# francois141/nori-ray-tracer

Measured on AMD Instinct MI355X. Metric: Msamples/sec on cbox_path_mis 512×512@512spp; per-pixel L2 vs CPU ref, higher is better.
Workload: dtype f32; 1 GPU; cbox_path_mis 512x512@512spp; scene=scenes/pa4/cbox/cbox_path_mis.xml, integrator=path_mis, parallelism=single GPU

## Files before the change

include/nori_gpu.h:

```cpp
#ifndef NORI_GPU_H
#define NORI_GPU_H

#ifndef __HIPCC_RTC__
#include <stddef.h>
#endif
#include <stdint.h>

#ifdef __cplusplus
extern "C" {
#endif

#define NORI_GPU_ABI_VERSION 7

#define NORI_OK               0
#define NORI_ERR_INVALID     -1
#define NORI_ERR_IO          -2
#define NORI_ERR_PARSE       -3
#define NORI_ERR_UNSUPPORTED -4
#define NORI_ERR_HIP         -5
#define NORI_ERR_CANCELLED   -6
#define NORI_ERR_OOM         -7

enum { NORI_SHAPE_MESH = 0 , NORI_SHAPE_SPHERE = 1  };
enum {
// ... 172 lines not shown
int nori_read_exr(const char *path, int *width, int *height, float *rgb);
int nori_read_image(const char *path, int *width, int *height, uint8_t *rgb);

typedef struct nori_bvh_info {
    uint32_t ref_nodes;
    uint32_t device_nodes;
    uint32_t depth;
    uint32_t num_prims;
    float sah_cost;
    uint32_t pad;
    uint64_t order_hash;
} nori_bvh_info;
int nori_scene_bvh_info(const nori_scene_desc *scene, nori_bvh_info *out);

typedef struct nori_scan_info {
    uint32_t records;
    uint32_t pairs;
    uint32_t plane_end[3];
    uint32_t tris;
} nori_scan_info;
int nori_scene_scan_list(const nori_scene_desc *scene, nori_scan_info *info, float *records, float *plane_c,
                         float *plane_f);

int nori_scene_scan_rtc(const nori_scene_desc *scene, const char *arch, size_t *code_bytes, double *ms);

int nori_scene_shade_rtc(const nori_scene_desc *scene, const char *arch, size_t *code_bytes, double *ms);

typedef struct nori_gpu_ctx nori_gpu_ctx;

typedef struct nori_gpu_render_desc {
    uint32_t pass_begin;
    uint32_t pass_count;
    uint32_t num_blocks;
    const uint32_t *block_ids;
    uint64_t seed;
    int32_t output_on_device;
    uint32_t path_pool;
    int32_t timing;
    float *variance_out;
} nori_gpu_render_desc;

typedef struct nori_gpu_stats {
    uint64_t samples;
    uint64_t invalid_samples;
    uint64_t rays_closest;
    uint64_t rays_shadow;
// ... 170 lines not shown
```

nori-ray-tracer_amd/csrc/kernels.h:

```cpp
#pragma once
#include <hip/hip_runtime.h>

#include <string>
#include <vector>

#include "film_put.h"
#include "kernel_config.h"

namespace nori {

constexpr int kTraceBlock = 128;
constexpr int kTraceSpill = 64;
#ifndef NORI_STACK_KEYS
#define NORI_STACK_KEYS 1
#endif
constexpr int stack_lds_entries(int stack) { return NORI_STACK_KEYS ? stack / 2 : stack; }
constexpr int kSplatBlock = 256;
#ifndef NORI_SCATTER_ROWS
#define NORI_SCATTER_ROWS 1
#endif
#ifndef NORI_SCAN_RAYS
#define NORI_SCAN_RAYS 2
#endif
constexpr int kScanRays = NORI_SCAN_RAYS;
#ifndef NORI_SCAN_RAYS_SHADOW
#define NORI_SCAN_RAYS_SHADOW 1
#endif
constexpr int kScanRaysShadow = NORI_SCAN_RAYS_SHADOW;

struct SplatDesc {
    uint32_t M;
    uint32_t passes;
    uint32_t pass_begin;
    uint32_t passes_per_wg;
    const int4 *blocks;
    uint64_t seed;
    float *var;
};

struct ScanRtcScene {
    const float *rec;
    uint32_t nrec;
    const float *plane_c, *plane_f;
    uint32_t pairs;
    uint32_t plane_end[3];
    uint32_t tris, real;
};
struct ScanRtc {
    hipModule_t mod = nullptr;
    hipFunction_t extend = nullptr, shadow = nullptr, trace[2] = {nullptr, nullptr};
    hipFunction_t both = nullptr;
    int k_extend = 0;
    double compile_ms = 0.0;
    bool cached = false;
    size_t code_bytes = 0;
};
struct ShadeRtc {
    hipModule_t mod = nullptr;
    hipFunction_t shade = nullptr;
    int integrator = 0;
    bool lds = false;
    double compile_ms = 0.0;
    bool cached = false;
    size_t code_bytes = 0;
};
constexpr bool kShadeRtcDefault = true;
std::string rtc_const_scene(const ScanRtcScene &sc);
bool rtc_compile(const ScanRtcScene &sc, const std::string &arch, int trace_cull, std::vector<char> &code, double &ms,
                 bool &cached, std::string &why, bool fresh = false);
// ... 91 lines not shown
```

nori-ray-tracer_amd/csrc/rtc.hip:

```cpp
#include <dlfcn.h>
#include <sys/stat.h>
#include <unistd.h>

#include <cerrno>
#include <chrono>
#include <cstdio>
#include <cstdlib>
#include <cstring>
#include <map>
#include <mutex>
#include <string>
#include <vector>

#include "kernels.h"
#include "rtc_cache.h"
#include "shade_kernel.h"

namespace nori {

#include "rtc_headers.inc"

namespace {

bool rtc_debug() {
// ... 219 lines not shown

bool rtc_off() {
    const char *e = std::getenv("NORI_RTC");
    return e && e[0] == '0';
}

}

int rtc_rays_per_thread() {
    const char *e = std::getenv("NORI_RTC_K");
    const int k = e ? std::atoi(e) : 1;
    return k == 1 || k == 2 || k == 4 ? k : 1;
}

std::string rtc_const_scene(const ScanRtcScene &sc) {
    std::string s = "#pragma once\n";
    s += "constexpr uint32_t kCPlaneEnd[3] = {" + std::to_string(sc.plane_end[0]) + "u, " +
         std::to_string(sc.plane_end[1]) + "u, " + std::to_string(sc.plane_end[2]) + "u};\n";
    s += "constexpr uint32_t kCTris = " + std::to_string(sc.tris) + "u, kCReal = " + std::to_string(sc.real) +
         "u, kCPrims = " + std::to_string(sc.nrec) + "u;\n";
    s += "constexpr float kCRec[] = {" + flt_list(sc.rec, 12 * (size_t)sc.nrec) + "};\n";
    s += "constexpr float kCPlaneF[] = {" + flt_list(sc.plane_f, 8 * (size_t)sc.pairs) + "};\n";
    s += "constexpr float kCPlaneC[] = {" + flt_list(sc.plane_c, sc.pairs) + "};\n";
    return s;
}

bool rtc_compile(const ScanRtcScene &sc, const std::string &arch, int trace_cull, std::vector<char> &code,
                 double &ms, bool &cached, std::string &why, bool fresh) {
    const int k = rtc_rays_per_thread();
    const char *wv = std::getenv("NORI_RTC_WAVES");
    RtcJob job{"scan_", "nori_scan_rtc.hip", kProgram, rtc_const_scene(sc), {
        "--offload-arch=" + arch, "-O3", "-std=c++17", "-ffp-contract=off", "-fno-slp-vectorize",
        "-munsafe-fp-atomics", "-DNORI_CONST_SCENE=1", "-DNORI_RTC_K=" + std::to_string(k),
        "-DNORI_RTC_WAVES=" + std::to_string(wv ? std::atoi(wv) : 0),
        "-DNORI_RTC_KS=" + std::to_string(kScanRaysShadow), "-DNORI_EXTEND_BLOCK=" + std::to_string(NORI_EXTEND_BLOCK),
        "-DNORI_SHADOW_BLOCK=" + std::to_string(NORI_SHADOW_BLOCK), "-DNORI_RTC_TRACE_BLOCK=" + std::to_string(kTraceBlock),
        "-DNORI_SCAN_GROUP=" + std::to_string(kScanGroup), "-DNORI_TRACE_GROUP=" + std::to_string(kTraceGroup),
        "-DNORI_SPHERE_FAST=" + std::to_string(NORI_SPHERE_FAST), "-DNORI_RTC_TRACE_CULL=" + std::to_string(trace_cull)}};
    return rtc_run(job, fresh, code, ms, cached, why);
}

bool rtc_compile_shade(const ScanRtcScene &sc, const std::string &arch, int integrator, bool lds,
                       std::vector<char> &code, double &ms, bool &cached, std::string &why, bool fresh) {
    RtcJob job{"shade_", "nori_shade_rtc.hip", kShadeProgram, rtc_const_scene(sc), {
        "--offload-arch=" + arch, "-O3", "-std=c++17", "-ffp-contract=off", "-fno-slp-vectorize",
        "-munsafe-fp-atomics", "-DNORI_CONST_SCENE=1", "-DNORI_RTC_INTEG=" + std::to_string(integrator),
// ... 130 lines not shown
```

nori-ray-tracer_amd/csrc/scan.h:

```cpp
#pragma once
#include "dev_scene.h"

namespace nori {

#define INF_F __builtin_inff()

struct TRay {
    V3 o, d, rcp;
    float mint, maxt;
};

ND bool box_test(const float4 &mn, const float4 &mx, const TRay &r, float &tnear) {
    bool ok = true;
    float nearT = -INF_F, farT = INF_F;
#define NORI_AXIS(c)                                                            \
    {                                                                           \
        float t1 = (mn.c - r.o.c) * r.rcp.c, t2 = (mx.c - r.o.c) * r.rcp.c;      \
        float lo = t1 > t2 ? t2 : t1, hi = t1 > t2 ? t1 : t2;                   \
        bool zero = r.d.c == 0.0f;                                              \
        float n2 = smax(lo, nearT), f2 = smin(hi, farT);                        \
        ok = ok && (zero ? !(r.o.c < mn.c || r.o.c > mx.c) : (n2 <= f2));       \
        nearT = zero ? nearT : n2;                                              \
        farT = zero ? farT : f2;                                                \
    }
    NORI_AXIS(x) NORI_AXIS(y) NORI_AXIS(z)
#undef NORI_AXIS
    tnear = nearT;
    return ok && r.mint <= farT && nearT <= r.maxt;
}

ND float rcp_det(float x) { return rcp_rn(x); }
ND bool tri_hit(const float4 &a, const float4 &b, const float4 &c, const TRay &r, float &t, float &u, float &v) {
    V3 v0 = ld3(a), e1 = ld3(b), e2 = ld3(c);
    V3 pvec = cross(r.d, e2);
    float det = dot(e1, pvec);
    if (det > -1e-8f && det < 1e-8f) return false;
    float inv_det = rcp_rn(det);
    V3 tvec = r.o - v0;
    u = dot(tvec, pvec) * inv_det;
    if (u < 0.0f || u > 1.0f) return false;
    V3 qvec = cross(tvec, e1);
    v = dot(r.d, qvec) * inv_det;
    if (v < 0.0f || u + v > 1.0f) return false;
    t = dot(e2, qvec) * inv_det;
    return t >= r.mint && t <= r.maxt;
}

ND bool sphere_hit(const float4 &a, const float4 &b, const TRay &r, float &t) {
    V3 oc = r.o - ld3(a);
    float rad = b.x;
    float A = dot(r.d, r.d);
    float B = 2.0f * dot(oc, r.d);
    float C = dot(oc, oc) - rad * rad;
    float disc = (B * B - 4 * A * C);
// ... 45 lines not shown
        inv_det;
    return !(det > -1e-8f && det < 1e-8f) && !(u < 0.0f || u > 1.0f) && !(v < 0.0f || u + v > 1.0f) &&
           t >= r.mint && t <= r.maxt;
}
template <bool FAST = false>
ND bool sphere_hit_nb(const float4 &a, const float4 &b, const TRay &r, float &t) {
    V3 oc = r.o - ld3(a);
    float rad = b.x;
    float A = dot(r.d, r.d);
    float B = 2.0f * dot(oc, r.d);
    float C = dot(oc, oc) - rad * rad;
    float disc = (B * B - 4 * A * C);
    float delta = fsqrt<FAST>(B * B - 4 * A * C);
    float t1 = (-B - delta) / (2 * A), t2 = (-B + delta) / (2 * A);
    bool h1 = r.mint <= t1 && t1 <= r.maxt, h2 = r.mint <= t2 && t2 <= r.maxt;
    t = h1 ? t1 : t2;
    return (disc > 0) && (h1 || h2);
}

#ifndef NORI_SPHERE_FAST
#define NORI_SPHERE_FAST 1
#endif
ND bool in_range60(float x) { return fabsf(x) >= 0x1p-60f && fabsf(x) <= 0x1p60f; }
ND bool sphere_hit_fast(const float4 &a, const float4 &b, const TRay &r, float &t) {
    if (!NORI_SPHERE_FAST) return sphere_hit_nb(a, b, r, t);
    V3 oc = r.o - ld3(a);
    float rad = b.x;
    float A = dot(r.d, r.d);
    float B = 2.0f * dot(oc, r.d);
    float C = dot(oc, oc) - rad * rad;
    float disc = (B * B - 4 * A * C);
    const float y = 2 * A;
#ifdef __HIP_DEVICE_COMPILE__
    const float s0 = __builtin_amdgcn_sqrtf(disc);
    const float sd = __uint_as_float(__float_as_uint(s0) - 1u), su = __uint_as_float(__float_as_uint(s0) + 1u);
    const float rd = __builtin_fmaf(-sd, s0, disc), ru = __builtin_fmaf(-su, s0, disc);
    float delta = ru > 0.0f ? su : (rd <= 0.0f ? sd : s0);
    const float ry = rcp_rn(y);
    float x1 = -B - delta, x2 = -B + delta;
    float q1 = x1 * ry, q2 = x2 * ry;
    float t1 = __builtin_fmaf(__builtin_fmaf(-y, q1, x1), ry, q1), t2 = __builtin_fmaf(__builtin_fmaf(-y, q2, x2), ry, q2);
    const bool fast = disc >= 0x1p-96f && disc < 0x1p96f && in_range60(y) && in_range60(x1) && in_range60(x2);
    if (__builtin_expect(disc > 0 && !fast, 0)) {
        delta = sqrtf(B * B - 4 * A * C);
        t1 = (-B - delta) / (2 * A);
        t2 = (-B + delta) / (2 * A);
    }
#else
    float delta = sqrtf(B * B - 4 * A * C);
    float t1 = (-B - delta) / y, t2 = (-B + delta) / y;
#endif
    bool h1 = r.mint <= t1 && t1 <= r.maxt, h2 = r.mint <= t2 && t2 <= r.maxt;
    t = h1 ? t1 : t2;
    return (disc > 0) && (h1 || h2);
}

template <int K>
ND void scan_prologue(const DevScene &S, TRay (&r)[K], bool (&live)[K]) {
    const float4 rmn = make_float4(S.root_min[0], S.root_min[1], S.root_min[2], 0.f);
    const float4 rmx = make_float4(S.root_max[0], S.root_max[1], S.root_max[2], 0.f);
#pragma unroll
    for (int k = 0; k < K; ++k) {
        TRay &x = r[k];
        if (x.mint == kEps) x.mint = smax(x.mint, x.mint * smax(smax(fabsf(x.o.x), fabsf(x.o.y)), fabsf(x.o.z)));
        x.rcp = V3{rcp_full(x.d.x), rcp_full(x.d.y), rcp_full(x.d.z)};
        float tn;
        live[k] = live[k] && !(x.maxt < x.mint) && box_test(rmn, rmx, x, tn);
    }
}

constexpr float kPlaneLo = 1.0f - 0x1p-16f, kPlaneHi = 1.0f + 0x1p-16f;
ND bool plane_may_hit(float o, float d, float c, float mint, float maxt) {
    const float T = o - c, ad = fabsf(d);
    const float s = d > 0.0f ? -T : T;
    const float lo = mint > 0.0f ? mint * kPlaneLo * ad : -INF_F, hi = maxt > 0.0f ? maxt * kPlaneHi * ad : INF_F;
    return s > lo && s < hi;
}

template <int A>
ND float comp(const V3 &v) { return A == 0 ? v.x : A == 1 ? v.y : v.z; }

template <int A>
ND bool pair_candidate(const TRay &r, const float4 &f0, const float4 &f1, float mlo, float mhi, float so, float sd) {
    constexpr int B = (A + 1) % 3, C = (A + 2) % 3;
    const float tf = (f1.y - comp<A>(r.o)) * comp<A>(r.rcp);
    const float dB = __builtin_fmaf(tf, comp<B>(r.d), comp<B>(r.o) - f0.x);
    const float dC = __builtin_fmaf(tf, comp<C>(r.d), comp<C>(r.o) - f0.z);
    const float S = __builtin_fmaf(fabsf(tf), sd, so);
// ... 134 lines not shown
    }
    NORI_SC_UNROLL
    for (uint32_t i = nt; i < n; ++i) {
        if (ANY && all_done()) return;
        const float4 p0 = NORI_SC_PRIM(3 * i), p1 = NORI_SC_PRIM(3 * i + 1);
        const uint32_t pos = __float_as_uint(NORI_SC_PRIM(3 * i + 2).w);
#pragma unroll
        for (int k = 0; k < K; ++k) {
            float t = 0;
            const bool h = sphere_hit_fast(p0, p1, r[k], t);
            if (h && live[k] && (ANY || t != tb[k] || pos > lb[k])) {
                found[k] = true;
                if (!ANY) {
                    r[k].maxt = tb[k] = t;
                    ub[k] = vb[k] = 0.0f;
                    pb[k] = __float_as_uint(p0.w);
                    lb[k] = pos;
                }
            }
        }
    }
}

template <int K, bool ANY, int CULL = 1, bool ZMINT = false>
ND void scan_rays(const DevScene &S, TRay (&r)[K], bool (&live)[K], float (&tb)[K], uint32_t (&pb)[K],
                  float (&ub)[K], float (&vb)[K], bool (&found)[K]) {
    scan_core<K, ANY, CULL, ZMINT>(S, r, live, tb, pb, ub, vb, found);
}

ND void path_ray(const DevScene &S, const float4 &a, const float4 &b, TRay &r) {
    r.o = ld3(a);
    r.d = ld3(b);
    const bool cam = (__float_as_uint(b.w) & kCameraRay) != 0u;
    r.mint = cam ? S.near_clip * a.w : kEps;
    r.maxt = cam ? S.far_clip * a.w : INF_F;
}

ND void shadow_add(float4 *rec, const float4 &c) {
    const uint32_t w = __float_as_uint(c.w);
    const float4 L = rec[w];
    rec[w] = make_float4(L.x + c.x, L.y + c.y, L.z + c.z, L.w);
}

#ifndef NORI_EXTEND_BLOCK
#define NORI_EXTEND_BLOCK 256
#endif
#ifndef NORI_SHADOW_BLOCK
#define NORI_SHADOW_BLOCK 256
#endif
// ... 93 lines not shown
```

nori-ray-tracer_amd/csrc/scene_prep.cpp:

```cpp
#include "scene_prep.h"

#include <algorithm>
#include <cstdio>
#include <cstdlib>
#include <cstring>

#include "rebuild.h"

namespace nori {

std::string &last_error() {
    static thread_local std::string e;
    return e;
}
bool debug_log() {
    const char *e = std::getenv("NORI_DEBUG");
    return e && e[0] == '1';
}

static float filter_eval(const nori_camera_desc &c, float x) {
    switch (c.filter_type) {
    case NORI_FILTER_GAUSSIAN: {
        float alpha = -1.0f / (2.0f * c.filter_p0 * c.filter_p0);
        float v = std::exp(alpha * x * x) - std::exp(alpha * c.filter_radius * c.filter_radius);
// ... 247 lines not shown
            const int a = k ? C : B;
            const float mid = (float)(0.5 * (lo[a] + hi[a]));
            const double half = std::max(hi[a] - mid, mid - lo[a]);
            const double Kb = (K1 * V + 2.0 * E * gam(70) + std::ldexp(E, -23) + std::ldexp(std::fabs(mid), -22)) * 1.05;
            f[2 * k] = mid;
            f[2 * k + 1] = (float)up(up(half) + Kb);
        }
        f[4] = (float)up(Ka);
        f[5] = L.plane_c[g];
    }
}
static bool axis_plane(const float *r, int a) {
    const float *e1 = r + 4, *e2 = r + 8;
    if (e1[a] != 0.0f || e2[a] != 0.0f) return false;
    const int b = (a + 1) % 3, c = (a + 2) % 3;
    for (int k : {b, c}) {
        for (float x : {e1[k], e2[k]})
            if (x != 0.0f && !(std::fabs(x) >= 0x1p-60f && std::fabs(x) <= 0x1p60f)) return false;
    }
    const double P = (double)e1[b] * e2[c], Q = (double)e1[c] * e2[b];
    const double diff = std::fabs(P - Q);
    return diff > 0.0 && (std::fabs(P) + std::fabs(Q)) <= 32.0 * diff;
}
ScanList build_scan_list(const DeviceBvh &bvh, uint32_t n) {
    ScanList L;
    auto rec = [&](uint32_t i) { return &bvh.prims[12 * (size_t)i]; };
    auto sphere = [&](uint32_t i) {
        uint32_t f;
        std::memcpy(&f, rec(i) + 7, 4);
        return f != 0u;
    };
    auto add = [&](uint32_t i) {
        const float *r = rec(i);
        L.prims.insert(L.prims.end(), r, r + 12);
        std::memcpy(&L.prims[L.prims.size() - 1], &i, 4);
    };
    auto add_null = [&] {
        float null_prim[12] = {0};
        const uint32_t none = 0xFFFFFFFFu;
        std::memcpy(&null_prim[3], &none, 4);
        L.prims.insert(L.prims.end(), null_prim, null_prim + 12);
    };
    if (const char *e = std::getenv("NORI_PLANE_CULL"); e && e[0] == '0') {
        for (uint32_t i = 0; i < n; ++i)
            if (!sphere(i)) add(i), ++L.tris;
        L.real = L.tris;
        for (; L.tris % kScanListGroup; ++L.tris) add_null();
// ... 119 lines not shown
int nori_scene_scan_list(const nori_scene_desc *d, nori_scan_info *info, float *records, float *plane_c,
                         float *plane_f) {
    return guarded([&] {
        if (!d || !info) return fail(NORI_ERR_INVALID, "null argument");
        if (d->abi_version != NORI_GPU_ABI_VERSION) return fail(NORI_ERR_INVALID, "ABI version mismatch");
        float rmin[3], rmax[3];
        scene_root_box(*d, rmin, rmax);
        DeviceBvh bvh;
        build_device_bvh(*d, rmin, rmax, bvh);
        const uint32_t n = (uint32_t)(bvh.prims.size() / 12);
        std::memset(info, 0, sizeof(*info));
        if (n > kScanMaxPrims) return NORI_OK;
        const ScanList L = build_scan_list(bvh, n);
        info->records = (uint32_t)(L.prims.size() / 12);
        info->pairs = (uint32_t)L.plane_c.size();
        for (int a = 0; a < 3; ++a) info->plane_end[a] = L.plane_end[a];
        info->tris = L.tris;
        if (records) std::memcpy(records, L.prims.data(), L.prims.size() * 4);
        if (plane_c && !L.plane_c.empty()) std::memcpy(plane_c, L.plane_c.data(), L.plane_c.size() * 4);
        if (plane_f && !L.plane_f.empty()) std::memcpy(plane_f, L.plane_f.data(), L.plane_f.size() * 4);
        return NORI_OK;
    });
}
void nori_scene_free(nori_scene *s) { delete s; }

int nori_film_border(const nori_scene_desc *d) { return d ? film_border(d->camera) : NORI_ERR_INVALID; }
int nori_filter_table(const nori_scene_desc *d, float *table) {
    if (!d || !table) return fail(NORI_ERR_INVALID, "null argument");
    filter_table(d->camera, table);
    return NORI_OK;
}
int nori_film_develop(const nori_scene_desc *d, const float *rgbw, float *rgb) {
    if (!d || !rgbw || !rgb) return fail(NORI_ERR_INVALID, "null argument");
    int W = d->camera.width, H = d->camera.height, B = film_border(d->camera), FW = W + 2 * B;
    for (int y = 0; y < H; ++y)
        for (int x = 0; x < W; ++x) {
            const float *c = rgbw + 4 * ((size_t)(y + B) * FW + (x + B));
            float *o = rgb + 3 * ((size_t)y * W + x);
            for (int k = 0; k < 3; ++k) o[k] = c[3] != 0 ? c[k] / c[3] : 0.0f;
        }
    return NORI_OK;
}

int nori_scene_bvh_refit(const nori_scene_desc *d, const float *positions, float *nodes, float *prims, float *root_box) {
    return guarded([&] {
        if (!d) return fail(NORI_ERR_INVALID, "null argument");
// ... 46 lines not shown
```

nori-ray-tracer_amd/csrc/scene_prep.h:

```cpp
#pragma once
#include <cmath>
#include <exception>
#include <memory>
#include <new>
#include <string>
#include <vector>

#include "host_scene.h"

struct nori_scene {
    std::unique_ptr<nori::HostScene> hs;
};

namespace nori {

constexpr uint32_t kScanMaxPrims = 64;
constexpr size_t kBlobMaxBytes = 48 << 10;
#ifndef NORI_SCAN_GROUP
#define NORI_SCAN_GROUP 4
#endif
constexpr uint32_t kScanListGroup = NORI_SCAN_GROUP;

std::string &last_error();
inline int fail(int code, const std::string &m) {
// ... 14 lines not shown
}
bool debug_log();

void filter_table(const nori_camera_desc &c, float *t);
int film_border(const nori_camera_desc &c);
int jit_code_lookup(float radius, float lookup);

struct EnvTables {
    uint32_t rgb_off, pdf_off, cdf_off, pmarg_off, cmarg_off;
};
EnvTables build_envmap(const nori_emitter_desc &e, std::vector<float> &env);

std::vector<uint32_t> spiral_blocks(int W, int H);
void scene_root_box(const nori_scene_desc &d, float rmin[3], float rmax[3]);
std::vector<uint8_t> solitary_spheres(const nori_scene_desc &d, const float rmin[3], const float rmax[3]);

struct ScanList {
    std::vector<float> prims;
    std::vector<float> plane_c;
    std::vector<float> plane_f;
    uint32_t plane_end[3] = {0, 0, 0};
    uint32_t tris = 0;
    uint32_t real = 0;
};
ScanList build_scan_list(const DeviceBvh &bvh, uint32_t n);

bool basic_scene(const nori_scene_desc &d);

template <class Vtx> float mesh_area_cdf(const uint32_t *tri, uint32_t count, Vtx vtx, std::vector<float> &cdf) {
    cdf.assign((size_t)count + 1, 0.0f);
    for (uint32_t t = 0; t < count; ++t) {
        const uint32_t *f = tri + 3 * (size_t)t;
        const float *p0 = vtx(f[0]), *p1 = vtx(f[1]), *p2 = vtx(f[2]);
        float e1[3] = {p1[0] - p0[0], p1[1] - p0[1], p1[2] - p0[2]}, e2[3] = {p2[0] - p0[0], p2[1] - p0[1], p2[2] - p0[2]};
        float cx = e1[1] * e2[2] - e1[2] * e2[1], cy = e1[2] * e2[0] - e1[0] * e2[2], cz = e1[0] * e2[1] - e1[1] * e2[0];
        float area = 0.5f * std::sqrt((cx * cx + cy * cy) + cz * cz);
        cdf[t + 1] = cdf[t] + area;
    }
    const float sum = cdf[count];
    if (!(sum > 0)) return 0.0f;
    const float norm = 1.0f / sum;
    for (uint32_t t = 1; t <= count; ++t) cdf[t] *= norm;
    cdf[count] = 1.0f;
    return norm;
}

nori_gpu_render_desc shard_of(int W, int H, uint32_t spp, const nori_gpu_render_desc &whole, int mode, int nranks,
                              int rank, std::vector<uint32_t> &blocks);
// ... 6 lines not shown
```

nori-ray-tracer_amd/csrc/upload.hip:

```cpp
#include <algorithm>
#include <cmath>
#include <cstdio>
#include <cstdlib>
#include <cstring>
#include <memory>
#include <string>
#include <vector>

#include "bsdf_desc.h"
#include "ctx.h"

namespace nori {

static_assert(kScanListGroup == kScanGroup, "scene_prep.h and dev_scene.h disagree on NORI_SCAN_GROUP");

int bvh_stack_for(uint32_t depth, int forced) {
    const uint32_t need = 3 * depth + 1;
    int stack = 32;
    if (need <= (uint32_t)stack_lds_entries(8)) stack = 8;
    else if (need <= (uint32_t)stack_lds_entries(16) + kTraceSpill) stack = 16;
    if (forced) stack = forced;
    if (need > (uint32_t)stack_lds_entries(stack) + kTraceSpill) throw NoriException(NORI_ERR_UNSUPPORTED, "BVH too deep for the traversal stack");
    return stack;
}
// ... 1 lines not shown
namespace {

size_t scene_blob_bytes(const nori_scene_desc &d, size_t prim_floats, size_t node_floats) {
    size_t prims = 0, cdf = 0;
    for (uint32_t s = 0; s < d.num_shapes; ++s) {
        const bool mesh = d.shapes[s].type == NORI_SHAPE_MESH;
        prims += mesh ? d.shapes[s].tri_count : 1u;
        cdf += mesh ? (size_t)d.shapes[s].tri_count + 1 : 0u;
    }
    const size_t vtx = d.num_vertices ? d.num_vertices : 1u;
    const size_t parts[10] = {prim_floats * 4, prims * 12, vtx * 16, vtx * 16, prims * 4, d.num_shapes * sizeof(DevShape),
                              d.num_bsdfs * sizeof(DevBsdf), d.num_emitters * sizeof(DevEmitter), (cdf ? cdf : 1u) * 4,
                              node_floats * 4};
    size_t n = 0;
    for (size_t b : parts) n = (n + 15) / 16 * 16 + b;
    return (n + 15) / 16 * 16;
}
bool shade_rtc_scene(const nori_scene_desc &d, bool scan, size_t records) {
    return scan && records <= 2 * kScanMaxPrims && basic_scene(d) && d.integrator < NORI_INTEGRATOR_NORMALS;
}

ScanRtcScene rtc_scene_of(const ScanList &L) {
    return ScanRtcScene{L.prims.data(), (uint32_t)(L.prims.size() / 12), L.plane_c.data(), L.plane_f.data(),
                        (uint32_t)L.plane_c.size(), {L.plane_end[0], L.plane_end[1], L.plane_end[2]}, L.tris, L.real};
}

void upload_scene(nori_gpu_ctx &c, const nori_scene_desc &d) {
    std::vector<size_t> img_off(d.num_images);
    {
        std::vector<uint32_t> tex;
        for (uint32_t i = 0; i < d.num_images; ++i) {
            const nori_image_desc &im = d.images[i];
            if (!im.rgb || im.width <= 0 || im.height <= 0 || (im.wrap != NORI_WRAP_REPEAT && im.wrap != NORI_WRAP_CLAMP))
                throw NoriException(NORI_ERR_INVALID, "bad image description");
            img_off[i] = tex.size();
            const size_t n = (size_t)im.width * im.height;
            for (size_t t = 0; t < n; ++t)
                tex.push_back((uint32_t)im.rgb[3 * t] | ((uint32_t)im.rgb[3 * t + 1] << 8) | ((uint32_t)im.rgb[3 * t + 2] << 16));
        }
        if (tex.empty()) tex.assign(1, 0u);
        c.tex.upload(tex);
    }
    auto image_ptr = [&](int32_t i) -> const uint32_t * {
        if (i < 0) return nullptr;
        if ((uint32_t)i >= d.num_images) throw NoriException(NORI_ERR_INVALID, "image index out of range");
        return c.tex.as<uint32_t>() + img_off[i];
    };
// ... 492 lines not shown
```

nori-ray-tracer_amd/nori_amd/__init__.py:

```python
import ctypes as C
import os
import threading
import time

import numpy as np

from . import _abi
from ._abi import NoriError, check, lib

__all__ = ["load_scene", "Scene", "GpuRenderer", "RenderThread", "NoriError", "device_count",
           "develop", "write_exr", "write_png", "read_exr", "film_variance", "ldr_bytes", "variance_gray",
           "denoise", "read_image", "block_error", "film_features", "denoise_guided", "film_denoise_guided",
           "scene_surface", "bvh_refit", "bvh_rebuild", "film_splat"]


def _fptr(a):
    return a.ctypes.data_as(C.POINTER(C.c_float))


class Scene:

    def __init__(self, handle, path):
        self._h = C.c_void_p(handle)
        self.path = path
# ... 265 lines not shown
    info = _abi.BvhRebuildInfo()
    check(lib().nori_scene_bvh_rebuild(scene.desc_ptr, pp, leaf_max, qq, C.byref(info), None, None, None))
    nodes = np.zeros((info.device_nodes, 32), np.float32)
    prims = np.zeros((info.num_prims, 12), np.float32)
    box = np.zeros(6, np.float32)
    check(lib().nori_scene_bvh_rebuild(scene.desc_ptr, pp, leaf_max, qq, C.byref(info), _fptr(nodes), _fptr(prims),
                                       _fptr(box)))
    return nodes, prims, box, {k: getattr(info, k) for k in ("device_nodes", "depth", "num_prims", "leaf_max")}


class ScanInfo(C.Structure):
    _fields_ = [("records", C.c_uint32), ("pairs", C.c_uint32), ("plane_end", C.c_uint32 * 3), ("tris", C.c_uint32)]


def scan_list(scene):
    info = ScanInfo()
    check(lib().nori_scene_scan_list(scene.desc_ptr, C.byref(info), None, None, None))
    rec = np.zeros((info.records, 12), np.float32)
    pc = np.zeros(max(info.pairs, 1), np.float32)
    pf = np.zeros((max(info.pairs, 1), 8), np.float32)
    check(lib().nori_scene_scan_list(scene.desc_ptr, C.byref(info), _fptr(rec), _fptr(pc), _fptr(pf)))
    return {"records": rec, "plane_c": pc[:info.pairs], "plane_f": pf[:info.pairs],
            "plane_end": np.array(list(info.plane_end)), "tris": info.tris}


def scan_rtc(scene, arch="gfx950"):
    n, ms = C.c_size_t(), C.c_double()
    check(lib().nori_scene_scan_rtc(scene.desc_ptr, arch.encode(), C.byref(n), C.byref(ms)))
    return n.value, ms.value


def shade_rtc(scene, arch="gfx950"):
    n, ms = C.c_size_t(), C.c_double()
    check(lib().nori_scene_shade_rtc(scene.desc_ptr, arch.encode(), C.byref(n), C.byref(ms)))
    return n.value, ms.value


def read_exr(path):
    w, h = C.c_int(), C.c_int()
    check(lib().nori_read_exr(os.fsencode(path), C.byref(w), C.byref(h), None))
    out = np.zeros((h.value, w.value, 3), np.float32)
    check(lib().nori_read_exr(os.fsencode(path), C.byref(w), C.byref(h), _fptr(out)))
    return out


def read_image(path):
# ... 429 lines not shown
```

nori-ray-tracer_amd/nori_amd/_abi.py:

```python
import ctypes as C
import os

ABI_VERSION = 7

NORI_OK = 0
NORI_ERR_INVALID = -1
NORI_ERR_IO = -2
NORI_ERR_PARSE = -3
NORI_ERR_UNSUPPORTED = -4
NORI_ERR_HIP = -5
NORI_ERR_CANCELLED = -6
NORI_ERR_OOM = -7

SHAPE_MESH, SHAPE_SPHERE = 0, 1
BSDF_DIFFUSE, BSDF_MIRROR, BSDF_DIELECTRIC, BSDF_MICROFACET, BSDF_DISNEY = range(5)
EMITTER_AREA, EMITTER_ENVMAP, EMITTER_POINT, EMITTER_SPOT = 0, 1, 2, 3
TEXTURE_CONSTANT, TEXTURE_CHECKERBOARD, TEXTURE_IMAGE = 0, 1, 2
WRAP_REPEAT, WRAP_CLAMP = 0, 1
CAMERA_PERSPECTIVE, CAMERA_THINLENS, CAMERA_ADVANCED = 0, 1, 2
(INTEGRATOR_PATH_MATS, INTEGRATOR_PATH_MIS, INTEGRATOR_VOLUMETRIC, INTEGRATOR_NORMALS, INTEGRATOR_AV,
 INTEGRATOR_DIRECT, INTEGRATOR_DIRECT_EMS, INTEGRATOR_DIRECT_MATS, INTEGRATOR_DIRECT_MIS,
 INTEGRATOR_PHOTONMAPPER) = range(10)
INTEGRATOR_NAMES = {0: "path_mats", 1: "path_mis", 2: "volumetric", 3: "normals", 4: "av", 5: "direct",
                    6: "direct_ems", 7: "direct_mats", 8: "direct_mis", 9: "photonmapper"}
# ... 146 lines not shown
        return {k: getattr(self, k) for k, _ in self._fields_ if k != "reserved"}


SIGNATURES = {
    "nori_gpu_last_error": (C.c_char_p, []),
    "nori_gpu_abi_version": (C.c_int, []),
    "nori_scene_load_xml": (C.c_int, [C.c_char_p, C.c_int, C.c_int, C.c_int, C.POINTER(C.c_void_p)]),
    "nori_scene_get_desc": (C.POINTER(SceneDesc), [C.c_void_p]),
    "nori_scene_free": (None, [C.c_void_p]),
    "nori_film_border": (C.c_int, [C.POINTER(SceneDesc)]),
    "nori_filter_table": (C.c_int, [C.POINTER(SceneDesc), C.POINTER(C.c_float)]),
    "nori_film_develop": (C.c_int, [C.POINTER(SceneDesc), C.POINTER(C.c_float), C.POINTER(C.c_float)]),
    "nori_write_exr": (C.c_int, [C.c_char_p, C.POINTER(C.c_float), C.c_int, C.c_int]),
    "nori_write_png": (C.c_int, [C.c_char_p, C.POINTER(C.c_float), C.c_int, C.c_int]),
    "nori_film_variance": (C.c_int, [C.POINTER(SceneDesc), C.POINTER(C.c_float), C.POINTER(C.c_float)]),
    "nori_film_block_error": (C.c_int, [C.POINTER(SceneDesc), C.POINTER(C.c_float), C.POINTER(C.c_float)]),
    "nori_denoise": (C.c_int, [C.c_int, C.POINTER(C.c_float), C.POINTER(C.c_float), C.c_int, C.c_int, C.c_int,
                               C.c_int, C.c_float, C.c_int, C.POINTER(C.c_float)]),
    "nori_read_exr": (C.c_int, [C.c_char_p, C.POINTER(C.c_int), C.POINTER(C.c_int), C.POINTER(C.c_float)]),
    "nori_read_image": (C.c_int, [C.c_char_p, C.POINTER(C.c_int), C.POINTER(C.c_int), C.POINTER(C.c_uint8)]),
    "nori_scene_bvh_info": (C.c_int, [C.c_void_p, C.c_void_p]),
    "nori_scene_scan_list": (C.c_int, [C.c_void_p, C.c_void_p, C.POINTER(C.c_float), C.POINTER(C.c_float),
                                       C.POINTER(C.c_float)]),
    "nori_scene_scan_rtc": (C.c_int, [C.c_void_p, C.c_char_p, C.POINTER(C.c_size_t), C.POINTER(C.c_double)]),
    "nori_scene_shade_rtc": (C.c_int, [C.c_void_p, C.c_char_p, C.POINTER(C.c_size_t), C.POINTER(C.c_double)]),
    "nori_gpu_shade_rtc_info": (C.c_int, [C.c_void_p, C.POINTER(C.c_int), C.POINTER(C.c_int), C.POINTER(C.c_double),
                                          C.POINTER(C.c_size_t)]),
    "nori_gpu_device_count": (C.c_int, [C.POINTER(C.c_int)]),
    "nori_gpu_create": (C.c_int, [C.POINTER(SceneDesc), C.c_int, C.POINTER(C.c_void_p)]),
    "nori_gpu_render": (C.c_int, [C.c_void_p, C.POINTER(RenderDesc), C.c_void_p, C.POINTER(Stats)]),
    "nori_gpu_block_error": (C.c_int, [C.c_void_p, C.c_void_p, C.c_int, C.POINTER(C.c_float)]),
    "nori_gpu_render_adaptive": (C.c_int, [C.c_void_p, C.POINTER(RenderDesc), C.POINTER(AdaptiveDesc), C.c_void_p,
                                           C.POINTER(Stats)]),
    "nori_gpu_render_features": (C.c_int, [C.c_void_p, C.POINTER(RenderDesc), C.c_void_p, C.POINTER(Stats)]),
    "nori_film_features": (C.c_int, [C.POINTER(SceneDesc), C.POINTER(C.c_float), C.POINTER(C.c_float)]),
    "nori_film_denoise_guided": (C.c_int, [C.POINTER(C.c_float), C.POINTER(C.c_float), C.POINTER(C.c_float), C.c_int,
                                           C.c_int, C.POINTER(GuidedDesc), C.POINTER(C.c_float)]),
    "nori_denoise_guided": (C.c_int, [C.c_int, C.POINTER(C.c_float), C.POINTER(C.c_float), C.POINTER(C.c_float),
                                      C.c_int, C.c_int, C.POINTER(GuidedDesc), C.POINTER(C.c_float)]),
    "nori_gpu_trace": (C.c_int, [C.c_void_p, C.POINTER(C.c_float), C.c_uint32, C.c_int, C.POINTER(Hit)]),
    "nori_gpu_query": (C.c_int, [C.c_void_p, C.POINTER(QueryDesc), C.c_void_p, C.c_void_p, C.c_void_p,
                                 C.POINTER(Stats)]),
    "nori_scene_surface": (C.c_int, [C.POINTER(SceneDesc), C.c_uint32, C.POINTER(C.c_float), C.c_void_p, C.c_void_p]),
    "nori_gpu_camera_rays": (C.c_int, [C.c_void_p, C.POINTER(RenderDesc), C.c_void_p]),
    "nori_gpu_bsdf_eval": (C.c_int, [C.c_void_p, C.POINTER(ShadingDesc), C.c_void_p, C.c_void_p, C.c_void_p, C.c_void_p]),
    "nori_gpu_bsdf_sample": (C.c_int, [C.c_void_p, C.POINTER(ShadingDesc), C.c_void_p, C.c_void_p, C.c_void_p, C.c_void_p]),
# ... 15 lines not shown
                                         C.POINTER(BvhRebuildInfo), C.POINTER(C.c_float), C.POINTER(C.c_float),
                                         C.POINTER(C.c_float)]),
    "nori_gpu_rebuild_bvh": (C.c_int, [C.c_void_p, C.POINTER(RebuildDesc), C.POINTER(RebuildStats)]),
    "nori_gpu_cancel": (C.c_int, [C.c_void_p]),
    "nori_gpu_progress": (C.c_float, [C.c_void_p]),
    "nori_gpu_destroy": (None, [C.c_void_p]),
    "nori_gpu_comm_id": (C.c_int, [C.POINTER(C.c_ubyte)]),
    "nori_gpu_comm_create": (C.c_int, [C.POINTER(C.c_ubyte), C.c_int, C.c_int, C.c_int, C.POINTER(C.c_void_p)]),
    "nori_gpu_comm_rank": (C.c_int, [C.c_void_p, C.POINTER(C.c_int), C.POINTER(C.c_int)]),
    "nori_gpu_comm_destroy": (None, [C.c_void_p]),
    "nori_gpu_comm_library": (C.c_char_p, []),
    "nori_gpu_shard_desc": (C.c_int, [C.POINTER(SceneDesc), C.POINTER(RenderDesc), C.c_int, C.c_int, C.c_int,
                                      C.POINTER(RenderDesc), C.POINTER(C.c_uint32)]),
    "nori_gpu_render_sharded": (C.c_int, [C.c_void_p, C.c_void_p, C.POINTER(RenderDesc), C.c_int, C.c_int,
                                          C.c_void_p, C.POINTER(Stats)]),
    "nori_gpu_comm_status_word": (C.c_int, [C.c_int, C.c_int]),
    "nori_gpu_comm_timeout": (C.c_double, [C.c_int, C.c_double, C.c_double, C.c_double]),
}

ADDED_IN_7 = {"nori_gpu_query", "nori_scene_surface", "nori_gpu_camera_rays", "nori_gpu_update_vertices",
              "nori_gpu_bvh_read", "nori_scene_bvh_refit", "nori_scene_bvh_rebuild", "nori_gpu_rebuild_bvh",
              "nori_scene_shade_rtc", "nori_gpu_shade_rtc_info", "nori_gpu_bsdf_eval", "nori_gpu_bsdf_sample",
              "nori_gpu_emitter_sample", "nori_gpu_emitter_eval", "nori_gpu_sample_uniforms", "nori_film_splat",
              "nori_gpu_film_splat", "nori_gpu_film_splat_passes"}

COMM_ID_BYTES = 128
SHARD_PASSES, SHARD_BLOCKS = 0, 1
SHARD_MODES = {"passes": SHARD_PASSES, "blocks": SHARD_BLOCKS}

PKG_DIR = os.path.dirname(os.path.dirname(os.path.abspath(__file__)))
LIB_PATH = os.environ.get("NORI_GPU_LIB") or os.path.join(PKG_DIR, "lib", "libnori_gpu.so")

_lib = None


def _one_hip_runtime():
    if os.environ.get("NORI_HIP_RUNTIME", "") == "system":
        return
    import importlib.util

    spec = importlib.util.find_spec("torch")
    if spec is None or not spec.origin:
        return
    tlib = os.path.join(os.path.dirname(spec.origin), "lib")
    for name in ("libhsa-runtime64.so", "libamdhip64.so"):
        path = os.path.join(tlib, name)
        if os.path.exists(path):
# ... 34 lines not shown
```

Before: 7580 Msamples/s.

## Specialize RTC scan on constant triangle edges with bounded-range fast reciprocals

For runtime-compiled constant scenes, adds a fast scan path that runs when every live ray's origin and direction magnitudes fall under a host-computed bound. Triangle tests are instantiated per primitive with literal edge vectors, so compile-time zero components drop their multiplies. Division uses a hardware reciprocal with one Newton refinement step instead of the correctly rounded path, and the host derives the bound so intermediate values stay in the normal range. This removes ALU work and branches from the brute-force scan, but risks slightly different rounding and larger generated code, and rays outside the bound fall back to the original path.

```diff
diff --git a/include/nori_gpu.h b/include/nori_gpu.h
--- a/include/nori_gpu.h
+++ b/include/nori_gpu.h
@@ -218,6 +218,8 @@
 int nori_scene_scan_list(const nori_scene_desc *scene, nori_scan_info *info, float *records, float *plane_c,
                          float *plane_f);
 
+int nori_scene_scan_fast(const nori_scene_desc *scene, float *fast_max);
+
 int nori_scene_scan_rtc(const nori_scene_desc *scene, const char *arch, size_t *code_bytes, double *ms);
 
 int nori_scene_shade_rtc(const nori_scene_desc *scene, const char *arch, size_t *code_bytes, double *ms);
diff --git a/nori-ray-tracer_amd/csrc/kernels.h b/nori-ray-tracer_amd/csrc/kernels.h
--- a/nori-ray-tracer_amd/csrc/kernels.h
+++ b/nori-ray-tracer_amd/csrc/kernels.h
@@ -45,6 +45,7 @@
     uint32_t pairs;
     uint32_t plane_end[3];
     uint32_t tris, real;
+    float fast_max;
 };
 struct ScanRtc {
     hipModule_t mod = nullptr;
diff --git a/nori-ray-tracer_amd/csrc/rtc.hip b/nori-ray-tracer_amd/csrc/rtc.hip
--- a/nori-ray-tracer_amd/csrc/rtc.hip
+++ b/nori-ray-tracer_amd/csrc/rtc.hip
@@ -265,6 +265,7 @@
     s += "constexpr float kCRec[] = {" + flt_list(sc.rec, 12 * (size_t)sc.nrec) + "};\n";
     s += "constexpr float kCPlaneF[] = {" + flt_list(sc.plane_f, 8 * (size_t)sc.pairs) + "};\n";
     s += "constexpr float kCPlaneC[] = {" + flt_list(sc.plane_c, sc.pairs) + "};\n";
+    s += "constexpr float kScanFastMax = " + flt(sc.fast_max) + ";\n";
     return s;
 }
 
diff --git a/nori-ray-tracer_amd/csrc/scan.h b/nori-ray-tracer_amd/csrc/scan.h
--- a/nori-ray-tracer_amd/csrc/scan.h
+++ b/nori-ray-tracer_amd/csrc/scan.h
@@ -30,6 +30,19 @@
 }
 
 ND float rcp_det(float x) { return rcp_rn(x); }
+ND float rcp_core(float x) {
+#ifdef __HIP_DEVICE_COMPILE__
+    const float r = __builtin_amdgcn_rcpf(x);
+    const float e = __builtin_fmaf(-x, r, 1.0f);
+    return __builtin_fmaf(e, r, r);
+#else
+    return 1.0f / x;
+#endif
+}
+ND float rcp_full_lo(float x) {
+    if (__builtin_expect(!(__builtin_fabsf(x) >= 0x1p-125f), 0)) return 1.0f / x;
+    return rcp_core(x);
+}
 ND bool tri_hit(const float4 &a, const float4 &b, const float4 &c, const TRay &r, float &t, float &u, float &v) {
     V3 v0 = ld3(a), e1 = ld3(b), e2 = ld3(c);
     V3 pvec = cross(r.d, e2);
@@ -121,6 +134,7 @@
 #define NORI_SPHERE_FAST 1
 #endif
 ND bool in_range60(float x) { return fabsf(x) >= 0x1p-60f && fabsf(x) <= 0x1p60f; }
+template <bool NOCHECK = false>
 ND bool sphere_hit_fast(const float4 &a, const float4 &b, const TRay &r, float &t) {
     if (!NORI_SPHERE_FAST) return sphere_hit_nb(a, b, r, t);
     V3 oc = r.o - ld3(a);
@@ -135,7 +149,9 @@
     const float sd = __uint_as_float(__float_as_uint(s0) - 1u), su = __uint_as_float(__float_as_uint(s0) + 1u);
     const float rd = __builtin_fmaf(-sd, s0, disc), ru = __builtin_fmaf(-su, s0, disc);
     float delta = ru > 0.0f ? su : (rd <= 0.0f ? sd : s0);
-    const float ry = rcp_rn(y);
+    float ry;
+    if constexpr (NOCHECK) ry = rcp_core(y);
+    else ry = rcp_rn(y);
     float x1 = -B - delta, x2 = -B + delta;
     float q1 = x1 * ry, q2 = x2 * ry;
     float t1 = __builtin_fmaf(__builtin_fmaf(-y, q1, x1), ry, q1), t2 = __builtin_fmaf(__builtin_fmaf(-y, q2, x2), ry, q2);
@@ -154,7 +170,7 @@
     return (disc > 0) && (h1 || h2);
 }
 
-template <int K>
+template <int K, bool BOUNDED = false>
 ND void scan_prologue(const DevScene &S, TRay (&r)[K], bool (&live)[K]) {
     const float4 rmn = make_float4(S.root_min[0], S.root_min[1], S.root_min[2], 0.f);
     const float4 rmx = make_float4(S.root_max[0], S.root_max[1], S.root_max[2], 0.f);
@@ -162,7 +178,8 @@
     for (int k = 0; k < K; ++k) {
         TRay &x = r[k];
         if (x.mint == kEps) x.mint = smax(x.mint, x.mint * smax(smax(fabsf(x.o.x), fabsf(x.o.y)), fabsf(x.o.z)));
-        x.rcp = V3{rcp_full(x.d.x), rcp_full(x.d.y), rcp_full(x.d.z)};
+        if constexpr (BOUNDED) x.rcp = V3{rcp_full_lo(x.d.x), rcp_full_lo(x.d.y), rcp_full_lo(x.d.z)};
+        else x.rcp = V3{rcp_full(x.d.x), rcp_full(x.d.y), rcp_full(x.d.z)};
         float tn;
         live[k] = live[k] && !(x.maxt < x.mint) && box_test(rmn, rmx, x, tn);
     }
@@ -343,9 +360,171 @@
     }
 }
 
+#ifdef NORI_CONST_SCENE
+ND bool scan_fast_ray(const TRay &r) {
+    const float s = ((((fabsf(r.o.x) + fabsf(r.o.y)) + fabsf(r.o.z)) + fabsf(r.d.x)) + fabsf(r.d.y)) + fabsf(r.d.z);
+    return s <= kScanFastMax && r.mint > 0.0f;
+}
+template <bool Z1, bool Z2>
+ND float diff_nz(float a, float k1, float b, float k2) {
+    if constexpr (Z1 && Z2) return 0.0f;
+    else if constexpr (Z1) return -(b * k2);
+    else if constexpr (Z2) return a * k1;
+    else return a * k1 - b * k2;
+}
+template <bool Z0, bool Z1, bool Z2>
+ND float sum_nz(float a, float b, float c) {
+    if constexpr (Z0 && Z1 && Z2) return 0.0f;
+    else if constexpr (Z0 && Z1) return c;
+    else if constexpr (Z0 && Z2) return b;
+    else if constexpr (Z1 && Z2) return a;
+    else if constexpr (Z0) return b + c;
+    else if constexpr (Z1) return a + c;
+    else if constexpr (Z2) return a + b;
+    else return (a + b) + c;
+}
+template <uint32_t I>
+ND bool tri_hit_lit(const TRay &r, float &t, float &u, float &v) {
+    constexpr float e1x = kCRec[12 * I + 4], e1y = kCRec[12 * I + 5], e1z = kCRec[12 * I + 6];
+    constexpr float e2x = kCRec[12 * I + 8], e2y = kCRec[12 * I + 9], e2z = kCRec[12 * I + 10];
+    constexpr bool a0 = e1x == 0.0f, a1 = e1y == 0.0f, a2 = e1z == 0.0f;
+    constexpr bool b0 = e2x == 0.0f, b1 = e2y == 0.0f, b2 = e2z == 0.0f;
+    constexpr bool p0 = b2 && b1, p1 = b0 && b2, p2 = b1 && b0;
+    constexpr bool q0 = a2 && a1, q1 = a0 && a2, q2 = a1 && a0;
+    const V3 d = r.d, tv = r.o - V3{kCRec[12 * I], kCRec[12 * I + 1], kCRec[12 * I + 2]};
+    const float px = diff_nz<b2, b1>(d.y, e2z, d.z, e2y), py = diff_nz<b0, b2>(d.z, e2x, d.x, e2z),
+                pz = diff_nz<b1, b0>(d.x, e2y, d.y, e2x);
+    const float det = sum_nz<a0 || p0, a1 || p1, a2 || p2>(e1x * px, e1y * py, e1z * pz);
+    const float inv_det = rcp_core(det);
+    u = sum_nz<p0, p1, p2>(tv.x * px, tv.y * py, tv.z * pz) * inv_det;
+    const float qx = diff_nz<a2, a1>(tv.y, e1z, tv.z, e1y), qy = diff_nz<a0, a2>(tv.z, e1x, tv.x, e1z),
+                qz = diff_nz<a1, a0>(tv.x, e1y, tv.y, e1x);
+    v = sum_nz<q0, q1, q2>(d.x * qx, d.y * qy, d.z * qz) * inv_det;
+    t = sum_nz<b0 || q0, b1 || q1, b2 || q2>(e2x * qx, e2y * qy, e2z * qz) * inv_det;
+    return (int)!((det > -1e-8f) & (det < 1e-8f)) & (int)!((u < 0.0f) | (u > 1.0f)) & (int)!((v < 0.0f) | (u + v > 1.0f)) &
+           (int)(t >= r.mint) & (int)(t <= r.maxt);
+}
+template <uint32_t I, int K, bool ANY>
+ND void scan_tri_lit(TRay (&r)[K], const bool (&live)[K], float (&tb)[K], uint32_t (&pb)[K], uint32_t (&lb)[K],
+                     float (&ub)[K], float (&vb)[K], bool (&found)[K]) {
+    constexpr bool e1_zero = kCRec[12 * I + 4] == 0.0f && kCRec[12 * I + 5] == 0.0f && kCRec[12 * I + 6] == 0.0f;
+    constexpr bool e2_zero = kCRec[12 * I + 8] == 0.0f && kCRec[12 * I + 9] == 0.0f && kCRec[12 * I + 10] == 0.0f;
+    if constexpr (!(e1_zero && e2_zero)) {
+        const uint32_t pos = __float_as_uint(kCRec[12 * I + 11]);
+#pragma unroll
+        for (int k = 0; k < K; ++k) {
+            float t = 0, u = 0, v = 0;
+            const bool h = tri_hit_lit<I>(r[k], t, u, v);
+            const bool take = (int)h & (int)live[k] & ((int)ANY | (int)(t != tb[k]) | (int)(pos > lb[k]));
+            found[k] = (int)found[k] | (int)take;
+            if (!ANY) {
+                r[k].maxt = take ? t : r[k].maxt;
+                tb[k] = take ? t : tb[k];
+                ub[k] = take ? u : ub[k];
+                vb[k] = take ? v : vb[k];
+                pb[k] = take ? __float_as_uint(kCRec[12 * I + 3]) : pb[k];
+                lb[k] = take ? pos : lb[k];
+            }
+        }
+    }
+}
+template <uint32_t G, uint32_t G1, int A, int K, bool ANY, int CULL>
+ND void scan_planes_lit(TRay (&r)[K], const bool (&live)[K], float (&tb)[K], uint32_t (&pb)[K], uint32_t (&lb)[K],
+                        float (&ub)[K], float (&vb)[K], bool (&found)[K]) {
+    if constexpr (G < G1) {
+        bool may = true;
+        if constexpr (CULL == 2) {
+            constexpr int B = (A + 1) % 3, C = (A + 2) % 3;
+            const float4 f0 = cpf(2 * G), f1 = cpf(2 * G + 1);
+            may = false;
+#pragma unroll
+            for (int k = 0; k < K; ++k) {
+                const float mlo = r[k].mint > 0.0f ? r[k].mint * kPlaneLo : -INF_F;
+                const float mhi = r[k].maxt > 0.0f ? r[k].maxt * kPlaneHi : INF_F;
+                const float so = fabsf(comp<B>(r[k].o)) + fabsf(comp<C>(r[k].o));
+                const float sd = fabsf(comp<B>(r[k].d)) + fabsf(comp<C>(r[k].d));
+                may = may || (live[k] && pair_candidate<A>(r[k], f0, f1, mlo, mhi, so, sd));
+            }
+        } else if constexpr (CULL != 0) {
+            may = false;
+#pragma unroll
+            for (int k = 0; k < K; ++k)
+                may = may || (live[k] && plane_may_hit(comp<A>(r[k].o), comp<A>(r[k].d), kCPlaneC[G], r[k].mint, r[k].maxt));
+        }
+        if (CULL == 0 || __any(may)) {
+            scan_tri_lit<2 * G, K, ANY>(r, live, tb, pb, lb, ub, vb, found);
+            scan_tri_lit<2 * G + 1, K, ANY>(r, live, tb, pb, lb, ub, vb, found);
+        }
+        scan_planes_lit<G + 1, G1, A, K, ANY, CULL>(r, live, tb, pb, lb, ub, vb, found);
+    }
+}
+template <int K>
+ND bool scan_all_done(const bool (&live)[K], const bool (&found)[K]) {
+    bool done = true;
+#pragma unroll
+    for (int k = 0; k < K; ++k) done = done && (found[k] || !live[k]);
+    return __all(done);
+}
+template <uint32_t I, int K, bool ANY>
+ND bool scan_rest_lit(TRay (&r)[K], const bool (&live)[K], float (&tb)[K], uint32_t (&pb)[K], uint32_t (&lb)[K],
+                      float (&ub)[K], float (&vb)[K], bool (&found)[K]) {
+    if constexpr (I < kCTris) {
+        if constexpr (ANY && (I - 2 * kCPlaneEnd[2]) % kScanGroup == 0)
+            if (scan_all_done<K>(live, found)) return true;
+        scan_tri_lit<I, K, ANY>(r, live, tb, pb, lb, ub, vb, found);
+        return scan_rest_lit<I + 1, K, ANY>(r, live, tb, pb, lb, ub, vb, found);
+    } else if constexpr (I < kCPrims) {
+        if (ANY && scan_all_done<K>(live, found)) return true;
+        const float4 p0 = crec(3 * I), p1 = crec(3 * I + 1);
+        const uint32_t pos = __float_as_uint(kCRec[12 * I + 11]);
+#pragma unroll
+        for (int k = 0; k < K; ++k) {
+            float t = 0;
+            const bool h = sphere_hit_fast<true>(p0, p1, r[k], t);
+            if (h && live[k] && (ANY || t != tb[k] || pos > lb[k])) {
+                found[k] = true;
+                if (!ANY) {
+                    r[k].maxt = tb[k] = t;
+                    ub[k] = vb[k] = 0.0f;
+                    pb[k] = __float_as_uint(p0.w);
+                    lb[k] = pos;
+                }
+            }
+        }
+        return scan_rest_lit<I + 1, K, ANY>(r, live, tb, pb, lb, ub, vb, found);
+    } else {
+        return false;
+    }
+}
+#endif
+
 template <int K, bool ANY, int CULL = 1, bool ZMINT = false>
 ND void scan_rays(const DevScene &S, TRay (&r)[K], bool (&live)[K], float (&tb)[K], uint32_t (&pb)[K],
                   float (&ub)[K], float (&vb)[K], bool (&found)[K]) {
+#ifdef NORI_CONST_SCENE
+    if constexpr (kScanFastMax > 0.0f) {
+        bool in = true;
+#pragma unroll
+        for (int k = 0; k < K; ++k) in = in && (!live[k] || scan_fast_ray(r[k]));
+        if (__builtin_expect(__all(in), 1)) {
+            scan_prologue<K, true>(S, r, live);
+            uint32_t lb[K];
+#pragma unroll
+            for (int k = 0; k < K; ++k) {
+                tb[k] = INF_F;
+                pb[k] = 0xFFFFFFFFu;
+                lb[k] = 0;
+                ub[k] = vb[k] = 0.0f;
+                found[k] = false;
+            }
+            scan_planes_lit<0, kCPlaneEnd[0], 0, K, ANY, CULL>(r, live, tb, pb, lb, ub, vb, found);
+            scan_planes_lit<kCPlaneEnd[0], kCPlaneEnd[1], 1, K, ANY, CULL>(r, live, tb, pb, lb, ub, vb, found);
+            scan_planes_lit<kCPlaneEnd[1], kCPlaneEnd[2], 2, K, ANY, CULL>(r, live, tb, pb, lb, ub, vb, found);
+            scan_rest_lit<2 * kCPlaneEnd[2], K, ANY>(r, live, tb, pb, lb, ub, vb, found);
+            return;
+        }
+    }
+#endif
     scan_core<K, ANY, CULL, ZMINT>(S, r, live, tb, pb, ub, vb, found);
 }
 
diff --git a/nori-ray-tracer_amd/csrc/scene_prep.cpp b/nori-ray-tracer_amd/csrc/scene_prep.cpp
--- a/nori-ray-tracer_amd/csrc/scene_prep.cpp
+++ b/nori-ray-tracer_amd/csrc/scene_prep.cpp
@@ -293,7 +293,35 @@
     const double diff = std::fabs(P - Q);
     return diff > 0.0 && (std::fabs(P) + std::fabs(Q)) <= 32.0 * diff;
 }
+static ScanList build_scan_list_(const DeviceBvh &bvh, uint32_t n);
+float scan_fast_max(const ScanList &L) {
+    if (const char *e = std::getenv("NORI_SCAN_FAST"); e && e[0] == '0') return 0.0f;
+    double E = 0.0, V = 0.0;
+    for (uint32_t i = 0; i < L.tris; ++i) {
+        const float *r = &L.prims[12 * (size_t)i];
+        for (int k = 0; k < 3; ++k) {
+            if (!std::isfinite(r[k]) || !std::isfinite(r[4 + k]) || !std::isfinite(r[8 + k])) return 0.0f;
+            V = std::max(V, std::fabs((double)r[k]));
+            E = std::max({E, std::fabs((double)r[4 + k]), std::fabs((double)r[8 + k])});
+        }
+    }
+    const double lim = std::ldexp(1.0, 125), slack = 1.0 + std::ldexp(1.0, -20);
+    auto fits = [&](double M) {
+        const double tv = M + V, pv = 2.0 * M * E, qv = 2.0 * tv * E;
+        const double worst = std::max({tv, pv, qv, 3.0 * E * pv, 3.0 * tv * pv, 3.0 * M * qv, 3.0 * E * qv, 6.0 * M * M});
+        return worst * slack <= lim;
+    };
+    double M = std::ldexp(1.0, 60);
+    while (M >= 1.0 && !fits(M)) M *= 0.5;
+    if (M < 1.0 || M < 16.0 * std::max(V, E)) return 0.0f;
+    return (float)M;
+}
 ScanList build_scan_list(const DeviceBvh &bvh, uint32_t n) {
+    ScanList L = build_scan_list_(bvh, n);
+    L.fast_max = scan_fast_max(L);
+    return L;
+}
+static ScanList build_scan_list_(const DeviceBvh &bvh, uint32_t n) {
     ScanList L;
     auto rec = [&](uint32_t i) { return &bvh.prims[12 * (size_t)i]; };
     auto sphere = [&](uint32_t i) {
@@ -459,6 +487,19 @@
         return NORI_OK;
     });
 }
+int nori_scene_scan_fast(const nori_scene_desc *d, float *fast_max) {
+    return guarded([&] {
+        if (!d || !fast_max) return fail(NORI_ERR_INVALID, "null argument");
+        if (d->abi_version != NORI_GPU_ABI_VERSION) return fail(NORI_ERR_INVALID, "ABI version mismatch");
+        float rmin[3], rmax[3];
+        scene_root_box(*d, rmin, rmax);
+        DeviceBvh bvh;
+        build_device_bvh(*d, rmin, rmax, bvh);
+        const uint32_t n = (uint32_t)(bvh.prims.size() / 12);
+        *fast_max = n > kScanMaxPrims ? 0.0f : build_scan_list(bvh, n).fast_max;
+        return NORI_OK;
+    });
+}
 void nori_scene_free(nori_scene *s) { delete s; }
 
 int nori_film_border(const nori_scene_desc *d) { return d ? film_border(d->camera) : NORI_ERR_INVALID; }
diff --git a/nori-ray-tracer_amd/csrc/scene_prep.h b/nori-ray-tracer_amd/csrc/scene_prep.h
--- a/nori-ray-tracer_amd/csrc/scene_prep.h
+++ b/nori-ray-tracer_amd/csrc/scene_prep.h
@@ -60,8 +60,10 @@
     uint32_t plane_end[3] = {0, 0, 0};
     uint32_t tris = 0;
     uint32_t real = 0;
+    float fast_max = 0.0f;
 };
 ScanList build_scan_list(const DeviceBvh &bvh, uint32_t n);
+float scan_fast_max(const ScanList &L);
 
 bool basic_scene(const nori_scene_desc &d);
 
diff --git a/nori-ray-tracer_amd/csrc/upload.hip b/nori-ray-tracer_amd/csrc/upload.hip
--- a/nori-ray-tracer_amd/csrc/upload.hip
+++ b/nori-ray-tracer_amd/csrc/upload.hip
@@ -47,7 +47,8 @@
 
 ScanRtcScene rtc_scene_of(const ScanList &L) {
     return ScanRtcScene{L.prims.data(), (uint32_t)(L.prims.size() / 12), L.plane_c.data(), L.plane_f.data(),
-                        (uint32_t)L.plane_c.size(), {L.plane_end[0], L.plane_end[1], L.plane_end[2]}, L.tris, L.real};
+                        (uint32_t)L.plane_c.size(), {L.plane_end[0], L.plane_end[1], L.plane_end[2]}, L.tris, L.real,
+                        L.fast_max};
 }
 
 void upload_scene(nori_gpu_ctx &c, const nori_scene_desc &d) {
diff --git a/nori-ray-tracer_amd/nori_amd/__init__.py b/nori-ray-tracer_amd/nori_amd/__init__.py
--- a/nori-ray-tracer_amd/nori_amd/__init__.py
+++ b/nori-ray-tracer_amd/nori_amd/__init__.py
@@ -311,6 +311,12 @@
     check(lib().nori_scene_scan_list(scene.desc_ptr, C.byref(info), _fptr(rec), _fptr(pc), _fptr(pf)))
     return {"records": rec, "plane_c": pc[:info.pairs], "plane_f": pf[:info.pairs],
             "plane_end": np.array(list(info.plane_end)), "tris": info.tris}
+
+
+def scan_fast_max(scene):
+    m = C.c_float()
+    check(lib().nori_scene_scan_fast(scene.desc_ptr, C.byref(m)))
+    return m.value
 
 
 def scan_rtc(scene, arch="gfx950"):
diff --git a/nori-ray-tracer_amd/nori_amd/_abi.py b/nori-ray-tracer_amd/nori_amd/_abi.py
--- a/nori-ray-tracer_amd/nori_amd/_abi.py
+++ b/nori-ray-tracer_amd/nori_amd/_abi.py
@@ -192,6 +192,7 @@
     "nori_scene_bvh_info": (C.c_int, [C.c_void_p, C.c_void_p]),
     "nori_scene_scan_list": (C.c_int, [C.c_void_p, C.c_void_p, C.POINTER(C.c_float), C.POINTER(C.c_float),
                                        C.POINTER(C.c_float)]),
+    "nori_scene_scan_fast": (C.c_int, [C.c_void_p, C.POINTER(C.c_float)]),
     "nori_scene_scan_rtc": (C.c_int, [C.c_void_p, C.c_char_p, C.POINTER(C.c_size_t), C.POINTER(C.c_double)]),
     "nori_scene_shade_rtc": (C.c_int, [C.c_void_p, C.c_char_p, C.POINTER(C.c_size_t), C.POINTER(C.c_double)]),
     "nori_gpu_shade_rtc_info": (C.c_int, [C.c_void_p, C.POINTER(C.c_int), C.POINTER(C.c_int), C.POINTER(C.c_double),
@@ -253,7 +254,7 @@
               "nori_gpu_bvh_read", "nori_scene_bvh_refit", "nori_scene_bvh_rebuild", "nori_gpu_rebuild_bvh",
               "nori_scene_shade_rtc", "nori_gpu_shade_rtc_info", "nori_gpu_bsdf_eval", "nori_gpu_bsdf_sample",
               "nori_gpu_emitter_sample", "nori_gpu_emitter_eval", "nori_gpu_sample_uniforms", "nori_film_splat",
-              "nori_gpu_film_splat", "nori_gpu_film_splat_passes"}
+              "nori_gpu_film_splat", "nori_gpu_film_splat_passes", "nori_scene_scan_fast"}
 
 COMM_ID_BYTES = 128
 SHARD_PASSES, SHARD_BLOCKS = 0, 1
```

Result: faster. 8046 Msamples/s (median of 6 runs) (+6.2%).
